# eMWu94/ReMo3D

Hardware: AMD Instinct MI355X
Metric: measurement points/sec (3D benchmark model) (higher is better)
Workload: dtype f64

## Files before the change

include/remo3d_hip_debug.h:

```cpp
#ifndef REMO3D_HIP_DEBUG_H
#define REMO3D_HIP_DEBUG_H

#include "remo3d_hip.h"

#ifdef __cplusplus
extern "C" {
#endif

int remo_debug_stream(remo_ctx_t *ctx, int64_t bytes, double *read_gbs, double *copy_gbs);
int remo_debug_clock(remo_ctx_t *ctx, double *gfma_per_wave);
int remo_debug_cache_gather(remo_ctx_t *ctx, int64_t bytes, double *gbs);
int remo_debug_device(remo_ctx_t *ctx, int64_t *out8);
int remo_debug_xcc(remo_ctx_t *ctx, int32_t *out, int32_t nblocks);


int remo_debug_patch_phases(remo_ctx_t *ctx, remo_batch_t *batch, int32_t fp32 , double *out16);

int remo_debug_patch_phases_p(remo_ctx_t *ctx, remo_batch_t *batch, int32_t fp32, double *out16);

int remo_debug_grid_barrier(remo_ctx_t *ctx, int32_t nblocks, int32_t nbar, double *out3);

int remo_debug_sens_timing(remo_ctx_t *ctx, double *out2);
int remo_debug_sens_group_timing(remo_ctx_t *ctx, double *out4);
int remo_debug_field_timing(remo_ctx_t *ctx, double *out2);
int remo_debug_point_location(remo_ctx_t *ctx);
int remo_debug_direction_bytes(remo_ctx_t *ctx);
int remo_debug_direction_forms(remo_ctx_t *ctx, int64_t n, int64_t nv, int32_t k, int32_t grid, int32_t step, double tol2, const double *r,
                               const float *p, const double *z, const double *dinv, const double *part_even, const double *part_odd,
                               int32_t nb_rz, const double *scal48, float *p_flat, float *p_row, double *scal_flat, double *scal_row);
int remo_debug_vector_heads(remo_ctx_t *ctx, int32_t on, double *out8);
int remo_debug_secondary_timing(remo_ctx_t *ctx, double *ms);
int remo_debug_pairs_timing(remo_ctx_t *ctx, double *out2);
int remo_debug_pair_groups_timing(remo_ctx_t *ctx, double *out4);

int remo_debug_tune(int32_t key, int32_t value);

#ifdef __cplusplus
}
#endif
#endif
```

remo3d_amd/_lib.py:

```python
from __future__ import annotations

import ctypes as C
import os

import numpy as np

_HERE = os.path.dirname(os.path.abspath(__file__))
LIB_PATH = os.environ.get("REMO_LIB") or os.path.join(_HERE, "libremo3d_hip.so")
REMO_MAX_RHS = 8


class RemoMesh(C.Structure):
    _fields_ = [("dim", C.c_int32), ("n_nodes", C.c_int64), ("coords", C.POINTER(C.c_double)),
                ("n_elems", C.c_int64), ("conn", C.POINTER(C.c_int32)), ("mat", C.POINTER(C.c_int32)),
                ("n_bfacets", C.c_int64), ("bconn", C.POINTER(C.c_int32)), ("bdirichlet", C.POINTER(C.c_uint8))]


class RemoOpts(C.Structure):
    _fields_ = [("preconditioner", C.c_int32), ("condense", C.c_int32), ("maxsteps", C.c_int32),
                ("check_every", C.c_int32), ("rtol", C.c_double), ("time_kernels", C.c_int32),
                ("coarse_degree", C.c_int32), ("coarse_ratio", C.c_int32), ("precision", C.c_int32), ("inner_digits", C.c_int32),
                ("serialize_solves", C.c_int32), ("op", C.c_int32), ("coarse", C.c_int32), ("assemble", C.c_int32), ("quadrature", C.c_int32)]


# ... 6 lines not shown
                ("spmv_ms", C.c_double), ("spmv_launches", C.c_int64), ("spmv_bytes", C.c_double),
                ("pcg_steps", C.c_int64), ("spmv_ms_raw", C.c_double), ("event_overhead_ms", C.c_double),
                ("refinement_cycles", C.c_int64), ("op_used", C.c_int32), ("coarse_used", C.c_int32),
                ("assembled", C.c_int32), ("patch_rounds", C.c_int32)]

    def as_dict(self):
        d = {}
        for name, _ in self._fields_:
            v = getattr(self, name)
            d[name] = list(v) if hasattr(v, "__len__") else v
        return d


class RemoJob(C.Structure):
    _dp, _ip = C.POINTER(C.c_double), C.POINTER(C.c_int32)
    _fields_ = [("size", C.c_uint32), ("tensor", C.c_int32), ("n_mat", C.c_int32), ("sigma", _dp),
                ("n_rhs", C.c_int32), ("src_ptr", _ip), ("src_p", _dp), ("src_I", _dp),
                ("eval_ptr", _ip), ("eval_p", _dp), ("u_out", _dp),
                ("n_fun", C.c_int32), ("fun_rhs", _ip), ("fun_ptr", _ip), ("fun_p", _dp), ("fun_w", _dp), ("J_out", _dp), ("dJ_out", _dp),
                ("n_group", C.c_int32), ("group", _ip), ("dJg_out", _dp),
                ("warm", C.c_void_p),
                ("n_pts", C.c_int32), ("pts", _dp), ("n_frhs", C.c_int32), ("field_rhs", _ip), ("u_f", _dp), ("grad_f", _dp), ("J_f", _dp),
                ("elem_f", _ip)]


class RemoJobSecondary(C.Structure):
    _fields_ = RemoJob._fields_ + [("secondary", C.c_int32), ("sec_quad", C.c_int32), ("sec_radius", C.c_double),
                                   ("sec_sigma0", C.POINTER(C.c_double))]


class RemoJobError(C.Structure):
    _fields_ = RemoJobSecondary._fields_ + [("err", C.c_int32), ("err_n_group", C.c_int32), ("err_group", C.POINTER(C.c_int32)),
                                            ("err_out", C.POINTER(C.c_double)), ("errg_out", C.POINTER(C.c_double))]


class RemoJobPairs(C.Structure):
    _fields_ = RemoJobError._fields_ + [("n_pair", C.c_int32), ("pair_reserved", C.c_int32), ("pair_a", C.POINTER(C.c_int32)),
                                        ("pair_b", C.POINTER(C.c_int32)), ("dP_out", C.POINTER(C.c_double))]


class RemoJobPairGroups(C.Structure):
    _fields_ = RemoJobPairs._fields_ + [("pair_n_group", C.c_int32), ("pair_group_reserved", C.c_int32), ("pair_group", C.POINTER(C.c_int32)),
                                        ("dPg_out", C.POINTER(C.c_double))]


EXPORTS = ["remo_abi_version", "remo_opts_default", "remo_ctx_create", "remo_ctx_destroy", "remo_last_error",
           "remo_solve_batch", "remo_solve_batch_tensor", "remo_solve_batch_sens", "remo_solve_batch_sens_tensor", "remo_solve_batch_sens_groups", "remo_solve_batch_sens_groups_tensor",
           "remo_solve_batch_field", "remo_solve_batch_field_tensor", "remo_batch_field", "remo_host_field_element",
           "remo_warm_create", "remo_warm_destroy", "remo_warm_clear", "remo_warm_info", "remo_solve_batch_sens_warm", "remo_solve_batch_sens_warm_tensor", "remo_batch_create", "remo_batch_create_tensor", "remo_batch_run", "remo_batch_fetch", "remo_batch_destroy",
           "remo_batch_eval", "remo_batch_get_system", "remo_batch_get_vectors", "remo_batch_apply_coarse", "remo_batch_spmv",
           "remo_host_element_matrix", "remo_host_element_matrix_tensor", "remo_host_sens_element", "remo_host_factor_error", "remo_host_symbolic",
           "remo_solve_job", "remo_batch_create_job", "remo_host_point_shapes", "remo_host_secondary_element", "remo_host_error_facet", "remo_host_pair_element"]
DEBUG_EXPORTS = ["remo_debug_stream", "remo_debug_clock", "remo_debug_device", "remo_debug_cache_gather", "remo_debug_xcc", "remo_debug_tune", "remo_debug_patch_phases", "remo_debug_patch_phases_p", "remo_debug_grid_barrier", "remo_debug_sens_timing", "remo_debug_sens_group_timing", "remo_debug_field_timing", "remo_debug_point_location", "remo_debug_secondary_timing", "remo_debug_direction_bytes", "remo_debug_pairs_timing", "remo_debug_pair_groups_timing",
                 "remo_debug_direction_forms", "remo_debug_vector_heads"]

JOB_HEAD = ["n_mat", "sigma", "n_rhs", "src_ptr", "src_p", "src_I", "eval_ptr", "eval_p"]
_SENS = ["u_out", "n_fun", "fun_rhs", "fun_ptr", "fun_p", "fun_w"]
LEGACY_MEMBERS = {"": ["u_out"],
                  "_sens": _SENS + ["J_out", "dJ_out"],
                  "_sens_warm": _SENS + ["J_out", "dJ_out", "warm"],
                  "_sens_groups": _SENS + ["n_group", "group", "J_out", "dJ_out", "dJg_out"],
                  "_field": ["u_out", "n_pts", "pts", "n_frhs", "field_rhs", "u_f", "grad_f", "J_f", "elem_f"]}


def legacy_args(job, kind=None):
    return [getattr(job, name) for name in JOB_HEAD + (LEGACY_MEMBERS[kind] if kind is not None else [])]


_lib = None


def load():
    global _lib
    if _lib is not None:
        return _lib
    if not os.path.exists(LIB_PATH):
        raise ImportError(f"{LIB_PATH} is missing: build it with `make -C remo3d_amd/csrc` "
                          "(or __graft_entry__.build()); remo3d_amd has no CPU fallback")
    L = C.CDLL(LIB_PATH)
    dp, ip, i64p, u8p = C.POINTER(C.c_double), C.POINTER(C.c_int32), C.POINTER(C.c_int64), C.POINTER(C.c_uint8)
    vp = C.c_void_p
    L.remo_abi_version.restype = C.c_int
    L.remo_opts_default.argtypes = [C.POINTER(RemoOpts)]
    L.remo_ctx_create.restype = vp
    L.remo_ctx_create.argtypes = [C.c_int]
    L.remo_ctx_destroy.argtypes = [vp]
    L.remo_last_error.restype = C.c_char_p
    L.remo_last_error.argtypes = [vp]
    member = dict(RemoJob._fields_)
    batch_args = [vp, C.POINTER(RemoMesh)] + [member[name] for name in JOB_HEAD]
    for kind, names in LEGACY_MEMBERS.items():
        for entry in (getattr(L, "remo_solve_batch" + kind), getattr(L, "remo_solve_batch" + kind + "_tensor")):
            entry.restype = C.c_int
            entry.argtypes = batch_args + [member[name] for name in names] + [C.POINTER(RemoOpts), C.POINTER(RemoStats)]
    L.remo_warm_create.restype = vp
    L.remo_warm_create.argtypes = [C.c_int]
    L.remo_warm_destroy.restype = None
    L.remo_warm_destroy.argtypes = [vp]
    L.remo_warm_clear.restype = None
    L.remo_warm_clear.argtypes = [vp]
    L.remo_warm_info.restype = C.c_int
    L.remo_warm_info.argtypes = [vp, i64p, ip, i64p, ip]
    L.remo_solve_job.restype = C.c_int
    L.remo_solve_job.argtypes = [vp, C.POINTER(RemoMesh), vp, C.POINTER(RemoOpts), C.POINTER(RemoStats)]
    L.remo_batch_create_job.restype = C.c_int
    L.remo_batch_create_job.argtypes = [vp, C.POINTER(RemoMesh), vp, C.POINTER(vp)]
    L.remo_host_point_shapes.restype = C.c_int
# ... 27 lines not shown
    L.remo_debug_sens_timing.restype = C.c_int
    L.remo_debug_sens_timing.argtypes = [vp, dp]
    L.remo_batch_create.restype = C.c_int
    L.remo_batch_create.argtypes = batch_args + [C.POINTER(vp)]
    L.remo_batch_create_tensor.restype = C.c_int
    L.remo_batch_create_tensor.argtypes = batch_args + [C.POINTER(vp)]
    L.remo_batch_run.restype = C.c_int
    L.remo_batch_run.argtypes = [vp, vp, C.POINTER(RemoOpts), C.POINTER(RemoStats)]
    L.remo_batch_fetch.restype = C.c_int
    L.remo_batch_fetch.argtypes = [vp, vp, dp]
    L.remo_batch_destroy.argtypes = [vp, vp]
    L.remo_batch_eval.restype = C.c_int
    L.remo_batch_eval.argtypes = [vp, vp, C.c_int32, C.c_int32, dp, dp]
    L.remo_batch_get_system.restype = C.c_int
    L.remo_batch_get_system.argtypes = [vp, vp, ip, ip, dp, dp, ip]
    L.remo_batch_get_vectors.restype = C.c_int
    L.remo_batch_get_vectors.argtypes = [vp, vp, dp, dp, ip]
    L.remo_batch_apply_coarse.restype = C.c_int
    L.remo_batch_apply_coarse.argtypes = [vp, vp, C.c_int32, dp, dp, C.c_int32, i64p]
    L.remo_debug_patch_phases.restype = C.c_int
    L.remo_debug_patch_phases.argtypes = [vp, vp, C.c_int32, dp]
    L.remo_debug_patch_phases_p.restype = C.c_int
    L.remo_debug_patch_phases_p.argtypes = [vp, vp, C.c_int32, dp]
    L.remo_debug_grid_barrier.restype = C.c_int
    L.remo_debug_grid_barrier.argtypes = [vp, C.c_int32, C.c_int32, dp]
    L.remo_debug_xcc.restype = C.c_int
    L.remo_debug_xcc.argtypes = [vp, ip, C.c_int32]
    L.remo_debug_cache_gather.restype = C.c_int
    L.remo_debug_cache_gather.argtypes = [vp, C.c_int64, dp]
    L.remo_debug_device.restype = C.c_int
    L.remo_debug_device.argtypes = [vp, i64p]
    L.remo_debug_clock.restype = C.c_int
    L.remo_debug_clock.argtypes = [vp, dp]
    L.remo_debug_stream.restype = C.c_int
    L.remo_debug_stream.argtypes = [vp, C.c_int64, dp, dp]
    L.remo_batch_spmv.restype = C.c_int
    L.remo_batch_spmv.argtypes = [vp, vp, C.c_int32, dp, dp, C.c_int32, dp]
    L.remo_host_element_matrix.restype = C.c_int
    L.remo_host_element_matrix.argtypes = [C.c_int32, dp, C.c_double, dp]
    L.remo_host_element_matrix_tensor.restype = C.c_int
    L.remo_host_element_matrix_tensor.argtypes = [C.c_int32, dp, dp, dp]
    L.remo_host_factor_error.restype = C.c_double
    L.remo_host_symbolic.restype = C.c_int
    L.remo_host_symbolic.argtypes = [C.POINTER(RemoMesh), C.c_int32, i64p, ip, ip, ip]
    L.remo_debug_tune.restype = C.c_int
    L.remo_debug_tune.argtypes = [C.c_int32, C.c_int32]
    fp = C.POINTER(C.c_float)
    if hasattr(L, "remo_debug_direction_forms"):
        L.remo_debug_direction_forms.restype = C.c_int
        L.remo_debug_direction_forms.argtypes = [vp, C.c_int64, C.c_int64, C.c_int32, C.c_int32, C.c_int32, C.c_double, dp, fp, dp, dp, dp, dp,
                                                 C.c_int32, dp, fp, fp, dp, dp]
        L.remo_debug_vector_heads.restype = C.c_int
        L.remo_debug_vector_heads.argtypes = [vp, C.c_int32, dp]
    _lib = L
    return L


def ptr(a, t):
    return a.ctypes.data_as(C.POINTER(t))


def mesh_struct(mesh):
    coords = np.ascontiguousarray(mesh.coords, dtype=np.float64)
    conn = np.ascontiguousarray(mesh.conn, dtype=np.int32)
    mat = np.ascontiguousarray(mesh.mat, dtype=np.int32)
    bconn = np.ascontiguousarray(mesh.bconn, dtype=np.int32).reshape(-1, mesh.dim)
    bdir = np.ascontiguousarray(mesh.bdirichlet, dtype=np.uint8)
    m = RemoMesh(int(mesh.dim), coords.shape[0], ptr(coords, C.c_double), conn.shape[0], ptr(conn, C.c_int32),
                 ptr(mat, C.c_int32), bconn.shape[0], ptr(bconn, C.c_int32), ptr(bdir, C.c_uint8))
    return m, (coords, conn, mat, bconn, bdir)
```

remo3d_amd/csrc/kernels.h:

```cpp
#pragma once
#include <hip/hip_runtime.h>
#include <stdint.h>

#include <type_traits>

#include "elem_access.h"
#include "tune.h"

namespace remo {

constexpr int kMaxPartialBlocks = 1024;
constexpr int kMaxPoints = 256;

template <int V> using int_c = std::integral_constant<int, V>;
template <class F> void for_k(int k, F &&fn) {
    switch (k) {
        case 1: fn(int_c<1>{}); break;
        case 2: fn(int_c<2>{}); break;
        case 3: fn(int_c<3>{}); break;
        case 4: fn(int_c<4>{}); break;
        case 5: fn(int_c<5>{}); break;
        case 6: fn(int_c<6>{}); break;
        case 7: fn(int_c<7>{}); break;
        default: fn(int_c<8>{}); break;
// ... 33 lines not shown
    const float *c32_ell_val = nullptr;
    float *c32_z = nullptr, *c32_res = nullptr, *c32_d[2] = {nullptr, nullptr};
    const AmgT<T> *amg = nullptr;
    const AmgT<float> *amg32 = nullptr;
    bool defer_q = false;
    bool x_in_direction = false;
    bool pq_bins = false;
    const int64_t *x_ev_at = nullptr;
    T *x_ev = nullptr;
    int x_ev_n = 0;
    float *p32 = nullptr;
    PcgProgress *progress;
    int progress_len;
    int nb_spmv, nb_vec;
};
using PcgBuffers = PcgBuffersT<double>;
constexpr int kPqBins = 256;
constexpr int kScalarSlots = 48;
constexpr int kDoneSlot = 4 * 8;

struct PatchTables {
    int64_t nt = 0, n = 0, npatch = 0;
    int E = 0;
    int rows_cap = 0;
    int block = 256;
    int trim = 1;
    int spread = 4;
    const uint16_t *lidx = nullptr;
    const int32_t *pcount = nullptr;
    const int32_t *prow = nullptr;
    const int32_t *pout = nullptr;
    const int32_t *pboff = nullptr;
    int all_slab = 1;
    const int32_t *row4 = nullptr;
    const int32_t *bptr = nullptr;
    const int32_t *bslot = nullptr;
    const double *C = nullptr;
    int64_t nslot_cap = 0;
    int stagger = 0;
    int rounds = 1;
};
template <class T> struct PatchOpT {
    PatchTables t;
    T *Yb = nullptr;
    double *ppart = nullptr;
    int lds_rows = 0;
    bool dot_bins = false;
};
#ifndef REMO_PATCH_PASSES
#define REMO_PATCH_PASSES 12
#endif
constexpr int kPatchPasses = REMO_PATCH_PASSES;
constexpr int kPatchBlock = 256;
inline size_t patch_lds_bytes(int lds_rows, int k) { return size_t(lds_rows + 2) * size_t(k) * 8; }
constexpr size_t kPatchLdsLimit = 63 * 1024;


template <class T> struct CsrViewT {
    int64_t n;
    int64_t nnz;
    const int32_t *rowptr;
    const int32_t *col;
    const T *val;
    int64_t pair_begin = 0, pair_end = 0;
    const PatchOpT<T> *patch = nullptr;
    bool vertex_block_only = false;
};
using CsrView = CsrViewT<double>;

void launch_metric_terms(const ElemMesh &em, int32_t *errflag, hipStream_t s);
void launch_metric_terms_tensor(const ElemMesh &em, int32_t *errflag, hipStream_t s);
void launch_diag_rows(int dim, int64_t row0, int64_t nfree, const int32_t *adjptr, const uint32_t *adj, const double *C, const double *M, double *dinv, hipStream_t s);
void launch_assemble(int dim, bool condense, int64_t nfree, int64_t pair_begin, int64_t pair_end, const int32_t *rowptr, const int32_t *col,
                     const int32_t *adjptr, const uint32_t *adj, const int32_t *eldof, const double *C,
                     const double *M, double *val, double *dinv, hipStream_t s);

int spmv_grid(int64_t n, int lanes_per_row);
int vec_grid(int64_t n);
int choose_lanes_per_row(int64_t n, int64_t nnz);
template <class T> bool patch_applies(const CsrViewT<T> &A, int k);
template <class T> void launch_spmm(const CsrViewT<T> &A, int k, const T *x, T *y, double *part, const double *scal, int nblocks, hipStream_t s, int step = 0, bool defer = false);

template <class T> void launch_patch_spmm(const CsrViewT<T> &A, int k, const T *x, T *y, double *part, const double *scal, int nblocks, hipStream_t s, int step, bool defer);
void launch_patch_spmm_x32(const CsrViewT<double> &A, int k, const float *x, double *part, const double *scal, int nblocks, hipStream_t s, int step);
template <class T> bool pcg_update_folds(const PcgBuffersT<T> &b);

template <class T> void launch_pcg_init(const CsrViewT<T> &A, int k, const T *f, const PcgBuffersT<T> &b, hipStream_t s);
template <class T> void launch_pcg_update(const CsrViewT<T> &A, int k, int step, double tol2, const PcgBuffersT<T> &b, hipStream_t s);
template <class T> void launch_pcg_direction(const CsrViewT<T> &A, int k, int step, double tol2, const PcgBuffersT<T> &b, hipStream_t s, bool add_x = true);
template <class T> void launch_pcg_final(int k, int step, const PcgBuffersT<T> &b, hipStream_t s);
void launch_direction_form(bool flat, int grid, int64_t n, int64_t nv, int k, int step, double tol2, int nb_rz, const double *part_rz_new,
                           double *scal, const double *r, float *p, const double *dinv, double *z, hipStream_t s);
void set_vector_stamps(long long *stamps);
void launch_vblock_bound(int64_t nv, const CsrView &A, const double *dinv, unsigned long long *out_bits, hipStream_t s);
constexpr int kSquareSlots = 512;
void launch_vblock_square(int64_t nv, const CsrView &A, const double *dinv, int32_t *sq_rowptr, int32_t *sq_col, double *sq_a, double *sq_b,
                          int64_t capacity, int32_t *flag, hipStream_t s);
int cheb_grid(int64_t nv);

void launch_barrier_probe(int nblocks, int nbar, unsigned *counter, int *fail, float *buf, int *mismatch, hipStream_t s);
constexpr int kEllWidth = 24;
void launch_vblock_ell(int64_t nv, const int32_t *rowptr, const int32_t *col, const double *val, int32_t *ecol, int32_t *tail, double *eval64,
                       float *eval32, hipStream_t s);


void launch_to_float(int64_t n, const double *src, float *dst, hipStream_t s);
void launch_vblock_compact(int64_t nv, const CsrView &A, int32_t *vb_rowptr, int32_t *vb_col, double *vb_val, int64_t capacity, int32_t *flag,
// ... 21 lines not shown
```

remo3d_amd/csrc/patch.h:

```cpp
#pragma once
#include "kernels.h"
#include "symbolic_gpu.h"

namespace remo {

size_t patch_arena_bytes(int64_t nt, int64_t n_max, int kmax);
void build_patch_tables(Arena &ar, hipStream_t s, const DeviceSymbolic &sy, const double *C, int kmax, int rounds, PatchTables &out, int32_t *flag_and_max);
int patch_rounds(int kmax, int wanted);
int patch_elements_per_group(int kmax, int rounds);
void set_patch_stamps(long long *device_buffer);

}
```

remo3d_amd/csrc/patch.hip:

```cpp
#include <hip/hip_runtime.h>
#include <limits.h>

#include <rocprim/device/device_scan.hpp>

#include "kernels.h"
#include "kutil.h"
#include "patch.h"
#include <stdexcept>
#include <type_traits>
#include "symbolic_gpu.h"
#include "wave_util.h"

#define REMO_ELEM_NS elem_tables_patch
#include "build/elem_apply.inc"

namespace remo {

namespace {

constexpr int kPatchDotBlocks = 32;
constexpr uint32_t kSlotBits = 13;
constexpr uint64_t kNoRow = uint64_t(0x7FFFFFFF);

__global__ void __launch_bounds__(256) k_patch_row_slots(int64_t n, int E, const int32_t *__restrict__ adjptr, const uint32_t *__restrict__ adj,
// ... 74 lines not shown
        if (lidx[j] == 0xFFFF) lidx[j] = z;
}

__global__ void __launch_bounds__(256) k_patch_slots(int E, int rows_cap, const int32_t *__restrict__ pcount, const int32_t *__restrict__ pboff,
                                                     const int32_t *__restrict__ prow, int32_t *__restrict__ pout, const int32_t *__restrict__ adjptr,
                                                     const uint32_t *__restrict__ adj, const int32_t *__restrict__ bptr, int32_t *__restrict__ bslot,
                                                     int32_t *__restrict__ row4) {
    const int64_t p = blockIdx.x;
    const int mp = pcount[p] < rows_cap ? pcount[p] : rows_cap;
    for (int m = threadIdx.x; m < mp; m += 256) {
        const int32_t row = prow[p * rows_cap + m], slot = pboff[p] + m;
        int32_t last = -1, rank = 0;
        for (int32_t a = adjptr[row]; a < adjptr[row + 1]; ++a) {
            const int32_t q = int32_t((adj[a] >> 5) / uint32_t(E));
            if (q >= p) break;
            rank += q != last;
            last = q;
        }
        pout[p * rows_cap + m] = slot;
        bslot[bptr[row] + rank] = slot;
        const int32_t cnt = bptr[row + 1] - bptr[row];
        if (rank < 3 || (rank == 3 && cnt <= 4)) row4[int64_t(row) * 4 + rank] = slot;
        else if (rank == 3) row4[int64_t(row) * 4 + 3] = -2;
    }
}

template <class T> __device__ __forceinline__ void lds_add(T *p, T v) {
    (void)__hip_atomic_fetch_add(p, v, __ATOMIC_RELAXED, __HIP_MEMORY_SCOPE_WORKGROUP);
}

#ifndef REMO_LEAN_WAVES
#define REMO_LEAN_WAVES 5
#endif
constexpr int kPatchPasses2 = 20;
template <class T, int K, int MODE = 0, bool LEAN = false, int ROUNDS = 1, class TX = T>
__global__ void __launch_bounds__(kPatchBlock, (LEAN ? REMO_LEAN_WAVES : 1)) k_patch_apply(PatchTables tb, int rows, const TX *__restrict__ x, T *__restrict__ y, T *__restrict__ Yb,
                                                     double *__restrict__ ppart, const double *__restrict__ scal, int step, long long *__restrict__ stamps,
                                                     double *__restrict__ pbins) {
    static_assert(std::is_same<TX, T>::value || (std::is_same<TX, float>::value && std::is_same<T, double>::value && MODE == 0 && !LEAN),
                  "an x narrower than the rest: fp32 into the fp64 product, plain order");
    (void)y;
    int done_word = 0;
    if (scal) done_word = load_as_vector(reinterpret_cast<const int *>(scal + kDoneSlot));
#define REMO_STAMP(k) if constexpr (MODE == 4) { if (threadIdx.x == 0) stamps[(int64_t(blockIdx.x) << 3) + (k)] = __builtin_readcyclecounter(); }
    REMO_STAMP(0)
    constexpr int NL = K;
    static_assert(ROUNDS == 1 || (ROUNDS == 2 && MODE == 0 && !LEAN), "two rounds: the plain order of the product only");
    constexpr int U = ROUNDS == 2 ? kPatchPasses2 : kPatchPasses;
    constexpr int BLK = kPatchBlock;
    constexpr int EK = BLK / K;
    constexpr uint32_t S = sizeof(T), SX = sizeof(TX);
    extern __shared__ double lds_raw[];
    TX *xs = reinterpret_cast<TX *>(lds_raw);
    __shared__ double smem[16 * K];
    const int tid = threadIdx.x;
    const int64_t per = (tb.npatch + 7) >> 3;
    const int64_t p = int64_t(blockIdx.x & 7) * per + int64_t(blockIdx.x >> 3);
    if (p >= tb.npatch) return;
    const int32_t *prow = tb.prow + p * tb.rows_cap;
    const int el = tid / NL, c0 = tid - el * NL;
    const int32_t off_mask = tid < EK * K ? 0 : int32_t(0x80000000);
    const rsrc_t rpr = make_rsrc(prow, uint64_t(tb.rows_cap) * 4);
    int32_t r0[U];
    const int rows_own_v = load_as_vector(tb.pcount + p);
    const int slab0_v = load_as_vector(tb.pboff + p);
#pragma unroll
    for (int u = 0; u < U; ++u) {
        int32_t t[1];
        buf_load<int32_t, 1>(rpr, off_mask == 0 ? uint32_t(el + EK * u) * 4u : kOutOfRange, t);
        r0[u] = t[0];
    }
    const int R = tb.spread > 1 ? tb.spread : 1;
    const int EL = ROUNDS == 2 ? (tb.E >> 1) : tb.E;
    const int run = el % R, base = EL / R, extra = EL % R;
    const int elp = R > 1 ? (run * base + (run < extra ? run : extra) + el / R) : el;
    const int64_t e = p * tb.E + elp;
    const bool active = el < EL && e < tb.nt;
    const int64_t eB = e + EL;
    const bool activeB = ROUNDS == 2 && el < EL && eB < tb.nt;
    uint32_t li[10];
    double cm[6];
#pragma unroll
    for (int q = 0; q < 10; ++q) li[q] = 0u;
#pragma unroll
    for (int q = 0; q < 6; ++q) cm[q] = 0.0;
    const rsrc_t rli = make_rsrc(tb.lidx, uint64_t(tb.nt) * 40), rcm = make_rsrc(tb.C, uint64_t(tb.nt) * 48);
    buf_load<uint32_t, 10>(rli, active ? uint32_t(e) * 40u : kOutOfRange, li);
    if constexpr (!(LEAN && MODE != 2)) buf_load<double, 6>(rcm, active ? uint32_t(e) * 48u : kOutOfRange, cm);
    uint32_t liB[ROUNDS == 2 ? 10 : 1];
    double cmB[ROUNDS == 2 ? 6 : 1];
    if constexpr (ROUNDS == 2) {
#pragma unroll
        for (int q = 0; q < 10; ++q) liB[q] = 0u;
#pragma unroll
        for (int q = 0; q < 6; ++q) cmB[q] = 0.0;
        buf_load<uint32_t, 10>(rli, activeB ? uint32_t(eB) * 40u : kOutOfRange, liB);
        buf_load<double, 6>(rcm, activeB ? uint32_t(eB) * 48u : kOutOfRange, cmB);
    }
    const int rows_own = __builtin_amdgcn_readfirstlane(rows_own_v);
    if (__builtin_amdgcn_readfirstlane(done_word) != 0 && __builtin_amdgcn_readfirstlane(done_word) <= step) return;
    const int rows_p = (tb.trim && rows_own < rows) ? rows_own : rows;
    const int npass = (rows_p + EK - 1) / EK;
    REMO_STAMP(1)
    const rsrc_t rx = make_rsrc(x, uint64_t(tb.n) * K * SX);
    const uint32_t slack = uint32_t((rows + 1) * K + c0);
#define REMO_PASSES_UP_TO_12(fn)                                                                                          \
        case 1: fn(std::integral_constant<int, 1>{}, 0); break;   case 2: fn(std::integral_constant<int, 2>{}, 0); break;   \
        case 3: fn(std::integral_constant<int, 3>{}, 0); break;   case 4: fn(std::integral_constant<int, 4>{}, 0); break;   \
        case 5: fn(std::integral_constant<int, 5>{}, 0); break;   case 6: fn(std::integral_constant<int, 6>{}, 0); break;   \
        case 7: fn(std::integral_constant<int, 7>{}, 0); break;   case 8: fn(std::integral_constant<int, 8>{}, 0); break;   \
        case 9: fn(std::integral_constant<int, 9>{}, 0); break;   case 10: fn(std::integral_constant<int, 10>{}, 0); break; \
        case 11: fn(std::integral_constant<int, 11>{}, 0); break; case 12: fn(std::integral_constant<int, 12>{}, 0); break;
#define REMO_PASSES(fn)                                                                                                   \
    if constexpr (ROUNDS == 2) {                                                                                          \
        switch (npass) {                                                                                                  \
            REMO_PASSES_UP_TO_12(fn)                                                                                      \
            case 13: fn(std::integral_constant<int, 13>{}, 0); break; case 14: fn(std::integral_constant<int, 14>{}, 0); break; \
            case 15: fn(std::integral_constant<int, 15>{}, 0); break; case 16: fn(std::integral_constant<int, 16>{}, 0); break; \
            case 17: fn(std::integral_constant<int, 17>{}, 0); break; case 18: fn(std::integral_constant<int, 18>{}, 0); break; \
            case 19: fn(std::integral_constant<int, 19>{}, 0); break; case 20: fn(std::integral_constant<int, 20>{}, 0); break; \
            default:                                                                                                      \
                for (int m0 = 0; m0 < rows_p; m0 += U * EK) fn(std::integral_constant<int, U>{}, m0);                     \
        }                                                                                                                 \
    } else {                                                                                                              \
        switch (npass) {                                                                                                  \
            REMO_PASSES_UP_TO_12(fn)                                                                                      \
            default:                                                                                                      \
                for (int m0 = 0; m0 < rows_p; m0 += U * EK) fn(std::integral_constant<int, U>{}, m0);                     \
        }                                                                                                                 \
    }
    static_assert(kPatchPasses == 12 && kPatchPasses2 == 20, "REMO_PASSES lists the cases 1 .. U");
    auto stage = [&](auto np_c, int m0) {
        constexpr int NP = decltype(np_c)::value;
        int32_t r[NP];
        TX v[NP][1];
        if (m0 == 0) {
#pragma unroll
            for (int u = 0; u < NP; ++u) r[u] = r0[u];
        } else {
#pragma unroll
            for (int u = 0; u < NP; ++u) {
                int32_t t[1];
                buf_load<int32_t, 1>(rpr, off_mask == 0 ? uint32_t(m0 + el + EK * u) * 4u : kOutOfRange, t);
                r[u] = t[0];
            }
        }
#pragma unroll
        for (int u = 0; u < NP; ++u) r[u] = (off_mask == 0 && m0 + el + EK * u < rows_own) ? r[u] : -1;
#pragma unroll
        for (int u = 0; u < NP; ++u)
            buf_load<TX, 1>(rx, r[u] >= 0 ? __umul24(uint32_t(r[u]), K * SX) + uint32_t(c0) * SX : kOutOfRange, v[u]);
#pragma unroll
        for (int u = 0; u < NP; ++u) xs[r[u] >= 0 ? uint32_t((m0 + el + EK * u) * K + c0) : slack] = v[u][0];
    };
    REMO_PASSES(stage)
    if (tid < 2 * K) xs[rows * K + tid] = TX(0);
    __syncthreads();
    REMO_STAMP(2)
    double d0 = 0.0;
    double *ya = lds_raw;
#define REMO_PATCH_L(i) ((li[(i) >> 1] >> (16 * ((i) & 1))) & 0xFFFFu)
    if constexpr (LEAN && MODE != 2) {
        typedef const T __attribute__((address_space(4))) *ctab_t;
        ctab_t tgi = (ctab_t)ElemTables2<T>::grad_in(), tdo = (ctab_t)ElemTables2<T>::div_out();
        if constexpr (sizeof(T) == 8) { asm volatile("" : "+s"(tgi)); asm volatile("" : "+s"(tdo)); }
        T g[30];
#define REMO_PATCH_XL(i) xs[REMO_PATCH_L(i) * K + c0]
#define REMO_BAR_ON __builtin_amdgcn_sched_barrier(0);
#define REMO_BAR_OFF
        if constexpr (sizeof(T) == 4) { REMO_ELEM_GRAD_IN(T, REMO_PATCH_XL, g, tgi, REMO_BAR_ON) }
        else { REMO_ELEM_GRAD_IN(T, REMO_PATCH_XL, g, tgi, REMO_BAR_OFF) }
#undef REMO_PATCH_XL
#pragma unroll
        for (int j = 0; j < 30; ++j) asm volatile("" : "+v"(g[j]));
        __builtin_amdgcn_sched_barrier(0);
        if (active) {
            const double *ce = tb.C + e * 6;
#pragma unroll
            for (int q = 0; q < 6; ++q) cm[q] = ce[q];
        }
        __syncthreads();
        REMO_STAMP(3)
        for (int j = 2 * tid; j < rows_p * K; j += 2 * BLK) { ya[j] = 0.0; ya[j + 1] = 0.0; }
        if (tid < K) ya[rows * K + tid] = 0.0;
        __syncthreads();
        REMO_STAMP(4)
        if (active) {
            const T c11 = T(cm[0]), c12 = T(cm[1]), c13 = T(cm[2]), c22 = T(cm[3]), c23 = T(cm[4]), c33 = T(cm[5]);
            T dd = T(0);
#pragma unroll
            for (int m = 0; m < 10; ++m) {
                const T g1 = g[m], g2 = g[10 + m], g3 = g[20 + m];
                const T h1 = c11 * g1 + c12 * g2 + c13 * g3, h2 = c12 * g1 + c22 * g2 + c23 * g3, h3 = c13 * g1 + c23 * g2 + c33 * g3;
                dd += g1 * h1 + g2 * h2 + g3 * h3;
                g[m] = h1; g[10 + m] = h2; g[20 + m] = h3;
            }
            d0 = double(dd);
            if constexpr (sizeof(T) == 8) {
                const uint32_t *pl2 = reinterpret_cast<const uint32_t *>(tb.lidx + e * 20);
#pragma unroll
                for (int q = 0; q < 10; ++q) li[q] = __builtin_nontemporal_load(pl2 + q);
            }
#define REMO_PATCH_EMIT(i, v) { if constexpr (MODE == 1) ya[REMO_PATCH_L(i) * K + c0] = double(v); else lds_add(ya + REMO_PATCH_L(i) * K + c0, double(v)); }
            if constexpr (sizeof(T) == 4) { REMO_ELEM_DIV_OUT(T, g, tdo, REMO_PATCH_EMIT, REMO_BAR_ON) }
            else { REMO_ELEM_DIV_OUT(T, g, tdo, REMO_PATCH_EMIT, REMO_BAR_OFF) }
#undef REMO_PATCH_EMIT
#undef REMO_BAR_ON
#undef REMO_BAR_OFF
        }
    } else if constexpr (ROUNDS == 2) {
        typedef const T __attribute__((address_space(4))) *ctab_t;
        ctab_t tgrad = (ctab_t)ElemTables<T>::grad(), tdiv = (ctab_t)ElemTables<T>::div();
        if constexpr (sizeof(T) == 8) { asm volatile("" : "+s"(tgrad)); asm volatile("" : "+s"(tdiv)); }
        auto element = [&](const T (&xe)[20], const double (&ce)[6], T (&ye)[20]) -> double {
            const T c11 = T(ce[0]), c12 = T(ce[1]), c13 = T(ce[2]), c22 = T(ce[3]), c23 = T(ce[4]), c33 = T(ce[5]);
            T g[30];
            REMO_ELEM_GRAD(T, xe, g, tgrad)
            T dd = T(0);
#pragma unroll
            for (int m = 0; m < 10; ++m) {
                const T g1 = g[m], g2 = g[10 + m], g3 = g[20 + m];
                const T h1 = c11 * g1 + c12 * g2 + c13 * g3, h2 = c12 * g1 + c22 * g2 + c23 * g3, h3 = c13 * g1 + c23 * g2 + c33 * g3;
                dd += g1 * h1 + g2 * h2 + g3 * h3;
                g[m] = h1; g[10 + m] = h2; g[20 + m] = h3;
            }
            REMO_ELEM_DIV(T, g, ye, tdiv)
            return double(dd);
        };
        auto emit = [&](int64_t ee, const T (&ye)[20]) {
            uint32_t lq[10];
            const uint32_t *pl2 = reinterpret_cast<const uint32_t *>(tb.lidx + ee * 20);
#pragma unroll
            for (int q = 0; q < 10; ++q) lq[q] = __builtin_nontemporal_load(pl2 + q);
#pragma unroll
            for (int i = 0; i < 20; ++i) lds_add(ya + ((lq[i >> 1] >> (16 * (i & 1))) & 0xFFFFu) * K + c0, double(ye[i]));
        };
        T yA[20], xB[20];
        double dA = 0.0;
        if (active) {
            T xA[20];
#pragma unroll
            for (int i = 0; i < 20; ++i) xA[i] = T(xs[REMO_PATCH_L(i) * K + c0]);
            dA = element(xA, cm, yA);
#pragma unroll
            for (int i = 0; i < 20; ++i) asm volatile("" : "+v"(yA[i]));
        }
        if (activeB) {
#pragma unroll
            for (int i = 0; i < 20; ++i) xB[i] = T(xs[((liB[i >> 1] >> (16 * (i & 1))) & 0xFFFFu) * K + c0]);
        }
        __syncthreads();
        REMO_STAMP(3)
        for (int j = 2 * tid; j < rows_p * K; j += 2 * BLK) { ya[j] = 0.0; ya[j + 1] = 0.0; }
        if (tid < K) ya[rows * K + tid] = 0.0;
        __syncthreads();
        REMO_STAMP(4)
        if (active) emit(e, yA);
        d0 = dA;
        if (activeB) {
            T yB[20];
            d0 += element(xB, cmB, yB);
            emit(eB, yB);
        }
    } else {
    T xv[20];
    if (active) {
#pragma unroll
        for (int i = 0; i < 20; ++i) xv[i] = T(xs[REMO_PATCH_L(i) * K + c0]);
    }
    __syncthreads();
    REMO_STAMP(3)
    for (int j = 2 * tid; j < rows_p * K; j += 2 * BLK) { ya[j] = 0.0; ya[j + 1] = 0.0; }
    if (tid < K) ya[rows * K + tid] = 0.0;
    __syncthreads();
    REMO_STAMP(4)
    if (active) {
        const T c11 = T(cm[0]), c12 = T(cm[1]), c13 = T(cm[2]), c22 = T(cm[3]), c23 = T(cm[4]), c33 = T(cm[5]);
        T g[30], yv[20];
        if constexpr (MODE == 2) {
#pragma unroll
            for (int i = 0; i < 20; ++i) yv[i] = xv[i] * c11;
        } else {
            typedef const T __attribute__((address_space(4))) *ctab_t;
            ctab_t tgrad = (ctab_t)ElemTables<T>::grad(), tdiv = (ctab_t)ElemTables<T>::div();
            if constexpr (sizeof(T) == 8) { asm volatile("" : "+s"(tgrad)); asm volatile("" : "+s"(tdiv)); }
            REMO_ELEM_GRAD(T, xv, g, tgrad)
            T dd = T(0);
#pragma unroll
            for (int m = 0; m < 10; ++m) {
                const T g1 = g[m], g2 = g[10 + m], g3 = g[20 + m];
                const T h1 = c11 * g1 + c12 * g2 + c13 * g3, h2 = c12 * g1 + c22 * g2 + c23 * g3, h3 = c13 * g1 + c23 * g2 + c33 * g3;
                dd += g1 * h1 + g2 * h2 + g3 * h3;
                g[m] = h1; g[10 + m] = h2; g[20 + m] = h3;
            }
            d0 = double(dd);
            REMO_ELEM_DIV(T, g, yv, tdiv)
        }
        {
            const uint32_t *pl2 = reinterpret_cast<const uint32_t *>(tb.lidx + e * 20);
// ... 194 lines not shown
    if constexpr (K == 5) {
        if (!launched && tb.rounds == 1 && mode >= 1 && mode <= 3 + (g_patch_stamps ? 1 : 0)) {
            launched = true;
            if (mode == 1) launch(k_patch_apply<T, 5, 1>);
            else if (mode == 2) launch(k_patch_apply<T, 5, 2>);
            else if (mode == 3) launch(k_patch_apply<T, 5, 3>);
            else launch(k_patch_apply<T, 5, 4>);
        }
    }
    if (!launched && tb.rounds == 1 && ((lean == 1) != (sizeof(T) == 4)) && lean >= 0) {
        if (sizeof(T) == 4) launch(k_patch_apply<T, K, 0>); else launch(k_patch_apply<T, K, 0, true>);
        launched = true;
    }
#endif
    if (!launched) {
        if constexpr (sizeof(T) == 4) {
            if (tb.rounds != 1) throw std::logic_error("patch operator: tables of two rounds in fp32 storage (they are built for fp64 solves only)");
            launch(k_patch_apply<T, K, 0, true>);
        } else {
            if (tb.rounds == 2) launch(k_patch_apply<T, K, 0, false, 2>);
            else launch(k_patch_apply<T, K, 0>);
        }
    }
    if (bins) return;
    if (part && defer) {
        hipLaunchKernelGGL(k_patch_dot<K>, dim3(nb < kPatchDotBlocks ? nb : kPatchDotBlocks), dim3(256), 0, s, tb.npatch, (const double *)P.ppart, part, scal, step);
        return;
    }
    if (part) hipLaunchKernelGGL((k_patch_reduce<T, K, true>), dim3(nb), dim3(256), 0, s, A.n, tb.npatch, tb.bptr, tb.bslot, (const T *)P.Yb, y, (const double *)P.ppart, part, scal, step);
    else hipLaunchKernelGGL((k_patch_reduce<T, K, false>), dim3(nb), dim3(256), 0, s, A.n, tb.npatch, tb.bptr, tb.bslot, (const T *)P.Yb, y, (const double *)nullptr, part, scal, step);
}

template <class T> void launch_patch_spmm(const CsrViewT<T> &A, int k, const T *x, T *y, double *part, const double *scal, int nb, hipStream_t s, int step, bool defer) {
    for_k(k, [&](auto kc) { constexpr int K = decltype(kc)::value; patch_dispatch<T, K>(A, x, y, part, scal, step, nb, s, defer); });
}
template <int K> static void patch_dispatch_x32(const CsrViewT<double> &A, const float *x, double *part, const double *scal, int step, int nb, hipStream_t s) {
    const PatchOpT<double> &P = *A.patch;
    const PatchTables &tb = P.t;
    const int64_t per = (tb.npatch + 7) / 8;
    double *bins = P.dot_bins ? part + (step & 1) * (kPqBins * 8) : nullptr;
    const size_t bytes = patch_lds_bytes(P.lds_rows, K);
    if (tb.rounds == 2)
        hipLaunchKernelGGL((k_patch_apply<double, K, 0, false, 2, float>), dim3(int(per * 8)), dim3(kPatchBlock), bytes, s, tb, P.lds_rows, x, (double *)nullptr, P.Yb, P.ppart, scal, step, (long long *)nullptr, bins);
    else
        hipLaunchKernelGGL((k_patch_apply<double, K, 0, false, 1, float>), dim3(int(per * 8)), dim3(kPatchBlock), bytes, s, tb, P.lds_rows, x, (double *)nullptr, P.Yb, P.ppart, scal, step, (long long *)nullptr, bins);
    if (!bins) hipLaunchKernelGGL(k_patch_dot<K>, dim3(nb < kPatchDotBlocks ? nb : kPatchDotBlocks), dim3(256), 0, s, tb.npatch, (const double *)P.ppart, part, scal, step);
}

void launch_patch_spmm_x32(const CsrViewT<double> &A, int k, const float *x, double *part, const double *scal, int nb, hipStream_t s, int step) {
    if (!patch_applies(A, k) || !part) throw std::logic_error("patch operator on an fp32 direction: no patch tables for this batch");
    for_k(k, [&](auto kc) { constexpr int K = decltype(kc)::value; patch_dispatch_x32<K>(A, x, part, scal, step, nb, s); });
}

template void launch_patch_spmm<double>(const CsrViewT<double> &, int, const double *, double *, double *, const double *, int, hipStream_t, int, bool);
template void launch_patch_spmm<float>(const CsrViewT<float> &, int, const float *, float *, double *, const double *, int, hipStream_t, int, bool);

}
```

remo3d_amd/csrc/remo_debug.hip:

```cpp
#include <limits.h>

#include <algorithm>
#include <vector>

#include "../../include/remo3d_hip_debug.h"
#include "remo_internal.h"
#include "patch.h"

using namespace remo;

namespace remo {
Tune g_tune;
}

extern "C" {

namespace {
__global__ void __launch_bounds__(256) k_stream_read(const double2 *__restrict__ x, int64_t n2, double *__restrict__ out) {
    double a = 0.0, b = 0.0;
    for (int64_t i = int64_t(blockIdx.x) * blockDim.x + threadIdx.x; i < n2; i += int64_t(gridDim.x) * blockDim.x) {
        const double2 v = x[i];
        a += v.x; b += v.y;
    }
    a += b;
// ... 240 lines not shown
};

int patch_probe_check(remo_ctx *ctx, remo_batch *b) {
    if (!b->has_system || b->run_id != ctx->run_id || !b->A.patch) return fail(ctx, REMO_ERR_ARG, "the last run on this batch did not use the patch operator");
    if (b->patch64.t.rounds != 1) return fail(ctx, REMO_ERR_ARG, "the batch's patch tables hold two elements per lane: set remo_debug_tune key 40 to 1 and run the batch again");
    if (PatchProbe::k * b->patch64.t.E > kPatchBlock) return fail(ctx, REMO_ERR_ARG, "the batch's patch tables are laid out for fewer than 5 columns");
    return REMO_OK;
}
}
#endif

int remo_debug_patch_phases(remo_ctx_t *ctx, remo_batch_t *b, int32_t fp32, double *out16) {
    if (!ctx || !b || !out16) return REMO_ERR_ARG;
#ifndef REMO_PROBES
    (void)fp32;
    return fail(ctx, REMO_ERR_ARG, "remo_debug_patch_phases: the library was built without -DREMO_PROBES (make -C remo3d_amd/csrc probes)");
#else
    if (int rc = patch_probe_check(ctx, b)) return rc;
    struct PersistOff { int was = g_tune.patch_persist; PersistOff() { g_tune.patch_persist = 0; } ~PersistOff() { g_tune.patch_persist = was; } } persist_off;
    try {
        HIP_TRY(hipSetDevice(ctx->device));
        const int64_t grid = (b->patch64.t.npatch + 7) / 8 * 8;
        std::vector<long long> h;
        {
            PatchProbe pr(ctx, b, fp32 != 0, size_t(grid) * 8);
            pr.stamped_runs();
            for (int mode = 0; mode <= 3; ++mode) {
                g_tune.patch_mode = mode;
                out16[10 + mode] = pr.timed_us();
            }
            g_tune.patch_mode = 0;
            h = pr.stamps();
        }
        for (int i = 0; i < 10; ++i) out16[i] = 0.0;
        long long lo = LLONG_MAX, hi = 0;
        int64_t cnt = 0;
        for (int64_t w = 0; w < grid; ++w) {
            const long long *s8 = h.data() + w * 8;
            if (s8[0] == 0 || s8[7] == 0) continue;
            for (int q = 0; q < 7; ++q) out16[q] += double(s8[q + 1] - s8[q]);
            out16[7] += double(s8[7] - s8[0]);
            lo = std::min(lo, s8[0]); hi = std::max(hi, s8[7]);
            ++cnt;
        }
        for (int q = 0; q < 8; ++q) out16[q] /= double(cnt > 0 ? cnt : 1);
        out16[8] = double(hi - lo);
        out16[9] = double(cnt);
        return REMO_OK;
    } catch (const std::exception &ex) {
        g_tune.patch_mode = 0; set_patch_stamps(nullptr);
        return fail(ctx, REMO_ERR_DEVICE, ex.what());
    }
#endif
}

int remo_debug_patch_phases_p(remo_ctx_t *ctx, remo_batch_t *b, int32_t fp32, double *out16) {
    if (!ctx || !b || !out16) return REMO_ERR_ARG;
#ifndef REMO_PROBES
    (void)fp32;
    return fail(ctx, REMO_ERR_ARG, "remo_debug_patch_phases_p: the library was built without -DREMO_PROBES (make -C remo3d_amd/csrc probes)");
#else
    if (int rc = patch_probe_check(ctx, b)) return rc;
    const int64_t slots = 8192;
    try {
        HIP_TRY(hipSetDevice(ctx->device));
        std::vector<long long> h;
        double us = 0.0;
        {
            PatchProbe pr(ctx, b, fp32 != 0, size_t(slots) * 12);
            pr.stamped_runs();
            us = pr.timed_us();
            h = pr.stamps();
        }
        for (int i = 0; i < 16; ++i) out16[i] = 0.0;
        double patches = 0, wgs = 0, longest = 0;
        for (int64_t w = 0; w < slots; ++w) {
            const long long *s12 = h.data() + w * 12;
            if (s12[10] <= 0) continue;
            double tot = 0;
            for (int q = 0; q < 10; ++q) { out16[q] += double(s12[q]); tot += double(s12[q]); }
            patches += double(s12[10]); wgs += 1; longest = std::max(longest, tot);
        }
        for (int q = 0; q < 10; ++q) out16[q] /= (patches > 0 ? patches : 1);
        out16[10] = patches; out16[11] = wgs; out16[12] = longest; out16[13] = us;
        return REMO_OK;
    } catch (const std::exception &ex) {
        g_tune.patch_mode = 0; set_patch_stamps(nullptr);
        return fail(ctx, REMO_ERR_DEVICE, ex.what());
    }
#endif
}

int remo_debug_direction_forms(remo_ctx_t *ctx, int64_t n, int64_t nv, int32_t k, int32_t grid, int32_t step, double tol2, const double *r,
                               const float *p, const double *z, const double *dinv, const double *part_even, const double *part_odd,
                               int32_t nb_rz, const double *scal48, float *p_flat, float *p_row, double *scal_flat, double *scal_row) {
    if (!ctx || n < 1 || nv < 0 || nv > n || k < 1 || k > 8 || grid < 1 || grid > kMaxPartialBlocks || step < 0 || nb_rz < 0 || nb_rz > kMaxPartialBlocks ||
        !r || !p || !dinv || (nv > 0 && !z) || !part_even || !part_odd || !scal48 || !p_flat || !p_row || !scal_flat || !scal_row)
        return REMO_ERR_ARG;
    if (uint64_t(n) * uint64_t(k) * 8 >= 0xFFFFF000ull) return fail(ctx, REMO_ERR_ARG, "remo_debug_direction_forms: n k sizeof(double) must stay below 4 GB (the flat form's range)");
    try {
        HIP_TRY(hipSetDevice(ctx->device));
        const size_t N = size_t(n) * k, NV = size_t(nv) * k, NP = size_t(nb_rz > 0 ? nb_rz : 1) * k;
        DeviceTemp tmp;
        double *dr = tmp.alloc<double>(N), *dz = tmp.alloc<double>(NV + 2), *dd = tmp.alloc<double>(n), *dpart = tmp.alloc<double>(2 * NP),
               *dscal = tmp.alloc<double>(48);
        float *dp = tmp.alloc<float>(N);
// ... 168 lines not shown
```

remo3d_amd/solver.py:

```python
from __future__ import annotations

import ctypes as C
from typing import Optional

import numpy as np

from . import _lib
from ._lib import RemoOpts, RemoStats, ptr

REMO_OK = 0
REMO_NOT_CONVERGED = 1
REMO_ERR_ARG = -1


class RemoError(RuntimeError):
    def __init__(self, code, msg):
        super().__init__(f"libremo3d_hip error {code}: {msg}")
        self.code = code


def make_opts(preconditioner="multigrid", condense=True, maxsteps=1000, rtol=1e-8, check_every=5,
              time_kernels=False, coarse_degree=0, coarse_ratio=0, precision="fp64", inner_digits=0,
              serialize_solves=False, op="auto", coarse="auto", quadrature="exact", assemble="auto") -> RemoOpts:
    L = _lib.load()
# ... 387 lines not shown
            n_group = int(groups.max(initial=-1)) + 1 if n_group is None else int(n_group)
            pg = (groups, n_group)
        out = self._one_shot("_sens", mesh, sigma, sources, evals, opts, raise_on_error, list(functionals) if functionals else [], pairs=pairs,
                             pair_groups=pg)
        if functionals:
            return out
        potentials, dP, st, rc = out[0], out[3], out[-2], out[-1]
        dPg = out[4] if pg is not None else None
        if far_field is not None and rc >= 0:
            ref = far_field_reference(mesh, sigma, float(far_field), *(pg or ()))
            c, dc = ref[0], ref[1]
            k = 2.0 if int(mesh.dim) == 3 else 1.0
            total = [float(np.sum(I)) for (_, I) in sources]
            potentials = [u + k * total[r] * c for r, u in enumerate(potentials)]
            if len(dP):
                pa, pb = _pair_arrays(pairs)
                kII = (k * np.array(total)[pa] * np.array(total)[pb]).reshape((-1,) + (1,) * dc.ndim)
                dP = dP + kII * dc[None]
                if pg is not None:
                    dPg = dPg + kII * ref[2][None]
        if pg is not None:
            return potentials, dP, dPg, st, rc
        return potentials, dP, st, rc

    def pairs_timing(self):
        out = np.zeros(2)
        self._L.remo_debug_pairs_timing(self._h, ptr(out, C.c_double))
        return float(out[0]), int(out[1])

    def pair_groups_timing(self):
        out = np.zeros(4)
        self._L.remo_debug_pair_groups_timing(self._h, ptr(out, C.c_double))
        return float(out[0]), float(out[1]), float(out[2]), int(out[3])

    def solve_batch_field(self, mesh, sigma, sources, evals, points, field_rhs=None, opts: Optional[RemoOpts] = None, raise_on_error=True):
        return self._one_shot("_field", mesh, sigma, sources, evals, opts, raise_on_error, points=points, field_rhs=field_rhs)

    def field_timing(self):
        out = np.zeros(2)
        self._L.remo_debug_field_timing(self._h, ptr(out, C.c_double))
        return float(out[0]), float(out[1])

    def secondary_timing(self) -> float:
        ms = C.c_double(0.0)
        self._L.remo_debug_secondary_timing(self._h, C.byref(ms))
        return float(ms.value)

    def point_location(self) -> int:
        return int(self._L.remo_debug_point_location(self._h))

    def direction_bytes(self) -> int:
        return int(self._L.remo_debug_direction_bytes(self._h))

    def sens_group_timing(self):
        out = np.zeros(4)
        self._L.remo_debug_sens_group_timing(self._h, ptr(out, C.c_double))
        return tuple(float(v) for v in out)

    def sens_timing(self):
        out = np.zeros(2)
        self._L.remo_debug_sens_timing(self._h, ptr(out, C.c_double))
        return float(out[0]), float(out[1])

    def batch(self, mesh, sigma, sources, evals, secondary=None) -> "Batch":
        return Batch(self, mesh, sigma, sources, evals, secondary)


class Batch:

    def __init__(self, ctx: Context, mesh, sigma, sources, evals, secondary=None):
        self.ctx = ctx
        self._L = ctx._L
        job = secondary is not None or _off_axis([z for (z, _) in sources], evals)
        if secondary is not None and not _secondary_members(secondary, len(sources))[3]:
            raise RemoError(REMO_ERR_ARG, "secondary: sigma0 must be positive and finite (None: the conductivity at the source)")
        (handle, ms, j), _, tensor, self._eval_ptr, keep = _batch_args(ctx._h, mesh, sigma, sources, evals, job, secondary)
        h = C.c_void_p()
        if job:
            rc = self._L.remo_batch_create_job(handle, ms, C.byref(j), C.byref(h))
        else:
            rc = (self._L.remo_batch_create_tensor if tensor else self._L.remo_batch_create)(handle, ms, *_lib.legacy_args(j), C.byref(h))
        if rc != 0:
            raise RemoError(rc, ctx.last_error())
        self._h = h
        self.dim = int(mesh.dim)
        self.n_rhs = len(sources)
        self.stats = None

    def run(self, opts: Optional[RemoOpts] = None, raise_on_error=True, ctx: Optional["Context"] = None):
        st = RemoStats()
        o = opts if opts is not None else make_opts()
        if ctx is not None:
            self.ctx = ctx
        rc = self._L.remo_batch_run(self.ctx._h, self._h, C.byref(o), C.byref(st))
        self.stats = st.as_dict()
        if rc < 0 and raise_on_error:
            raise RemoError(rc, self.ctx.last_error())
        return rc

    def fetch(self):
        eval_ptr = self._eval_ptr
        out = np.full(int(eval_ptr[-1]), np.nan)
        rc = self._L.remo_batch_fetch(self.ctx._h, self._h, ptr(out, C.c_double))
        if rc != 0:
            raise RemoError(rc, self.ctx.last_error())
        return [out[eval_ptr[k]:eval_ptr[k + 1]] for k in range(self.n_rhs)]
# ... 163 lines not shown
```

Measured before the change: 193.4.

## Alias patch smem into dynamic LDS and defer second-round loads to cut pressure

In the two-round patch apply kernel, the static 16*K shared scratch is dropped and aliased onto the dynamic LDS buffer, whose minimum size is raised to four rows so it can hold the scratch. The second-round index and coefficient loads are moved from the prologue to just before their use, with only a one-word cache warm-up issued early. Both changes aim to lower LDS and register footprint so more workgroups fit per CU, at the cost of exposing some load latency later in the kernel. A debug occupancy query export is also added.

```diff
diff --git a/include/remo3d_hip_debug.h b/include/remo3d_hip_debug.h
--- a/include/remo3d_hip_debug.h
+++ b/include/remo3d_hip_debug.h
@@ -15,6 +15,8 @@
 
 
 int remo_debug_patch_phases(remo_ctx_t *ctx, remo_batch_t *batch, int32_t fp32 , double *out16);
+
+int remo_debug_patch_occupancy(remo_ctx_t *ctx, int32_t lds_rows, int32_t k, int32_t rounds, int32_t x32, int32_t *out);
 
 int remo_debug_patch_phases_p(remo_ctx_t *ctx, remo_batch_t *batch, int32_t fp32, double *out16);
 
diff --git a/remo3d_amd/_lib.py b/remo3d_amd/_lib.py
--- a/remo3d_amd/_lib.py
+++ b/remo3d_amd/_lib.py
@@ -82,7 +82,7 @@
            "remo_host_element_matrix", "remo_host_element_matrix_tensor", "remo_host_sens_element", "remo_host_factor_error", "remo_host_symbolic",
            "remo_solve_job", "remo_batch_create_job", "remo_host_point_shapes", "remo_host_secondary_element", "remo_host_error_facet", "remo_host_pair_element"]
 DEBUG_EXPORTS = ["remo_debug_stream", "remo_debug_clock", "remo_debug_device", "remo_debug_cache_gather", "remo_debug_xcc", "remo_debug_tune", "remo_debug_patch_phases", "remo_debug_patch_phases_p", "remo_debug_grid_barrier", "remo_debug_sens_timing", "remo_debug_sens_group_timing", "remo_debug_field_timing", "remo_debug_point_location", "remo_debug_secondary_timing", "remo_debug_direction_bytes", "remo_debug_pairs_timing", "remo_debug_pair_groups_timing",
-                 "remo_debug_direction_forms", "remo_debug_vector_heads"]
+                 "remo_debug_direction_forms", "remo_debug_vector_heads", "remo_debug_patch_occupancy"]
 
 JOB_HEAD = ["n_mat", "sigma", "n_rhs", "src_ptr", "src_p", "src_I", "eval_ptr", "eval_p"]
 _SENS = ["u_out", "n_fun", "fun_rhs", "fun_ptr", "fun_p", "fun_w"]
@@ -216,6 +216,9 @@
                                                  C.c_int32, dp, fp, fp, dp, dp]
         L.remo_debug_vector_heads.restype = C.c_int
         L.remo_debug_vector_heads.argtypes = [vp, C.c_int32, dp]
+    if hasattr(L, "remo_debug_patch_occupancy"):
+        L.remo_debug_patch_occupancy.restype = C.c_int
+        L.remo_debug_patch_occupancy.argtypes = [vp, C.c_int32, C.c_int32, C.c_int32, C.c_int32, ip]
     _lib = L
     return L
 
diff --git a/remo3d_amd/csrc/kernels.h b/remo3d_amd/csrc/kernels.h
--- a/remo3d_amd/csrc/kernels.h
+++ b/remo3d_amd/csrc/kernels.h
@@ -109,7 +109,7 @@
 #endif
 constexpr int kPatchPasses = REMO_PATCH_PASSES;
 constexpr int kPatchBlock = 256;
-inline size_t patch_lds_bytes(int lds_rows, int k) { return size_t(lds_rows + 2) * size_t(k) * 8; }
+inline size_t patch_lds_bytes(int lds_rows, int k) { return size_t(lds_rows + 2 > 4 ? lds_rows + 2 : 4) * size_t(k) * 8; }
 constexpr size_t kPatchLdsLimit = 63 * 1024;
 
 
diff --git a/remo3d_amd/csrc/patch.h b/remo3d_amd/csrc/patch.h
--- a/remo3d_amd/csrc/patch.h
+++ b/remo3d_amd/csrc/patch.h
@@ -8,6 +8,7 @@
 void build_patch_tables(Arena &ar, hipStream_t s, const DeviceSymbolic &sy, const double *C, int kmax, int rounds, PatchTables &out, int32_t *flag_and_max);
 int patch_rounds(int kmax, int wanted);
 int patch_elements_per_group(int kmax, int rounds);
+int patch_apply_occupancy(int k, int rounds, bool x32, int lds_rows);
 void set_patch_stamps(long long *device_buffer);
 
 }
diff --git a/remo3d_amd/csrc/patch.hip b/remo3d_amd/csrc/patch.hip
--- a/remo3d_amd/csrc/patch.hip
+++ b/remo3d_amd/csrc/patch.hip
@@ -150,7 +150,12 @@
     constexpr uint32_t S = sizeof(T), SX = sizeof(TX);
     extern __shared__ double lds_raw[];
     TX *xs = reinterpret_cast<TX *>(lds_raw);
-    __shared__ double smem[16 * K];
+    double *smem;
+    if constexpr (ROUNDS == 2) smem = lds_raw;
+    else {
+        __shared__ double smem_static[16 * K];
+        smem = smem_static;
+    }
     const int tid = threadIdx.x;
     const int64_t per = (tb.npatch + 7) >> 3;
     const int64_t p = int64_t(blockIdx.x & 7) * per + int64_t(blockIdx.x >> 3);
@@ -185,15 +190,14 @@
     const rsrc_t rli = make_rsrc(tb.lidx, uint64_t(tb.nt) * 40), rcm = make_rsrc(tb.C, uint64_t(tb.nt) * 48);
     buf_load<uint32_t, 10>(rli, active ? uint32_t(e) * 40u : kOutOfRange, li);
     if constexpr (!(LEAN && MODE != 2)) buf_load<double, 6>(rcm, active ? uint32_t(e) * 48u : kOutOfRange, cm);
-    uint32_t liB[ROUNDS == 2 ? 10 : 1];
-    double cmB[ROUNDS == 2 ? 6 : 1];
+    uint32_t warmB[2] = {0u, 0u};
     if constexpr (ROUNDS == 2) {
-#pragma unroll
-        for (int q = 0; q < 10; ++q) liB[q] = 0u;
-#pragma unroll
-        for (int q = 0; q < 6; ++q) cmB[q] = 0.0;
-        buf_load<uint32_t, 10>(rli, activeB ? uint32_t(eB) * 40u : kOutOfRange, liB);
-        buf_load<double, 6>(rcm, activeB ? uint32_t(eB) * 48u : kOutOfRange, cmB);
+        uint32_t t[1];
+        const uint32_t eB0 = uint32_t(p * tb.E + EL), at = uint32_t(tid) * 16u;
+        buf_load<uint32_t, 1>(rli, at < uint32_t(EL) * 40u ? eB0 * 40u + at : kOutOfRange, t);
+        warmB[0] = t[0];
+        buf_load<uint32_t, 1>(rcm, at < uint32_t(EL) * 48u ? eB0 * 48u + at : kOutOfRange, t);
+        warmB[1] = t[0];
     }
     const int rows_own = __builtin_amdgcn_readfirstlane(rows_own_v);
     if (__builtin_amdgcn_readfirstlane(done_word) != 0 && __builtin_amdgcn_readfirstlane(done_word) <= step) return;
@@ -252,6 +256,7 @@
         for (int u = 0; u < NP; ++u) xs[r[u] >= 0 ? uint32_t((m0 + el + EK * u) * K + c0) : slack] = v[u][0];
     };
     REMO_PASSES(stage)
+    if constexpr (ROUNDS == 2) asm volatile("" : : "v"(warmB[0]), "v"(warmB[1]));
     if (tid < 2 * K) xs[rows * K + tid] = TX(0);
     __syncthreads();
     REMO_STAMP(2)
@@ -343,6 +348,15 @@
 #pragma unroll
             for (int i = 0; i < 20; ++i) asm volatile("" : "+v"(yA[i]));
         }
+        __builtin_amdgcn_sched_barrier(0);
+        uint32_t liB[10];
+        double cmB[6];
+#pragma unroll
+        for (int q = 0; q < 10; ++q) liB[q] = 0u;
+#pragma unroll
+        for (int q = 0; q < 6; ++q) cmB[q] = 0.0;
+        buf_load<uint32_t, 10>(rli, activeB ? uint32_t(eB) * 40u : kOutOfRange, liB);
+        buf_load<double, 6>(rcm, activeB ? uint32_t(eB) * 48u : kOutOfRange, cmB);
         if (activeB) {
 #pragma unroll
             for (int i = 0; i < 20; ++i) xB[i] = T(xs[((liB[i >> 1] >> (16 * (i & 1))) & 0xFFFFu) * K + c0]);
@@ -643,6 +657,24 @@
     for_k(k, [&](auto kc) { constexpr int K = decltype(kc)::value; patch_dispatch_x32<K>(A, x, part, scal, step, nb, s); });
 }
 
+int patch_apply_occupancy(int k, int rounds, bool x32, int lds_rows) {
+    int n = -1;
+    for_k(k, [&](auto kc) {
+        constexpr int K = decltype(kc)::value;
+        const size_t bytes = patch_lds_bytes(lds_rows, K);
+        hipError_t rc;
+        if (rounds == 2) {
+            if (x32) rc = hipOccupancyMaxActiveBlocksPerMultiprocessor(&n, k_patch_apply<double, K, 0, false, 2, float>, kPatchBlock, bytes);
+            else rc = hipOccupancyMaxActiveBlocksPerMultiprocessor(&n, k_patch_apply<double, K, 0, false, 2>, kPatchBlock, bytes);
+        } else {
+            if (x32) rc = hipOccupancyMaxActiveBlocksPerMultiprocessor(&n, k_patch_apply<double, K, 0, false, 1, float>, kPatchBlock, bytes);
+            else rc = hipOccupancyMaxActiveBlocksPerMultiprocessor(&n, k_patch_apply<double, K, 0>, kPatchBlock, bytes);
+        }
+        if (rc != hipSuccess) n = -1;
+    });
+    return n;
+}
+
 template void launch_patch_spmm<double>(const CsrViewT<double> &, int, const double *, double *, double *, const double *, int, hipStream_t, int, bool);
 template void launch_patch_spmm<float>(const CsrViewT<float> &, int, const float *, float *, double *, const double *, int, hipStream_t, int, bool);
 
diff --git a/remo3d_amd/csrc/remo_debug.hip b/remo3d_amd/csrc/remo_debug.hip
--- a/remo3d_amd/csrc/remo_debug.hip
+++ b/remo3d_amd/csrc/remo_debug.hip
@@ -316,6 +316,20 @@
         return fail(ctx, REMO_ERR_DEVICE, ex.what());
     }
 #endif
+}
+
+int remo_debug_patch_occupancy(remo_ctx_t *ctx, int32_t lds_rows, int32_t k, int32_t rounds, int32_t x32, int32_t *out) {
+    if (!ctx || !out || k < 1 || k > 8 || (rounds != 1 && rounds != 2) || lds_rows < 0) return REMO_ERR_ARG;
+    if (patch_lds_bytes(lds_rows, k) > kPatchLdsLimit) return fail(ctx, REMO_ERR_ARG, "remo_debug_patch_occupancy: more rows than a workgroup's LDS holds");
+    try {
+        HIP_TRY(hipSetDevice(ctx->device));
+        const int n = patch_apply_occupancy(k, rounds, x32 != 0, lds_rows);
+        if (n < 0) return fail(ctx, REMO_ERR_DEVICE, "hipOccupancyMaxActiveBlocksPerMultiprocessor failed");
+        *out = n;
+        return REMO_OK;
+    } catch (const std::exception &ex) {
+        return fail(ctx, REMO_ERR_DEVICE, ex.what());
+    }
 }
 
 int remo_debug_patch_phases_p(remo_ctx_t *ctx, remo_batch_t *b, int32_t fp32, double *out16) {
diff --git a/remo3d_amd/solver.py b/remo3d_amd/solver.py
--- a/remo3d_amd/solver.py
+++ b/remo3d_amd/solver.py
@@ -463,6 +463,13 @@
     def direction_bytes(self) -> int:
         return int(self._L.remo_debug_direction_bytes(self._h))
 
+    def patch_occupancy(self, lds_rows: int, k: int, rounds: int = 2, x32: bool = True) -> int:
+        out = C.c_int32(-1)
+        rc = self._L.remo_debug_patch_occupancy(self._h, int(lds_rows), int(k), int(rounds), 1 if x32 else 0, C.byref(out))
+        if rc != 0:
+            raise RemoError(rc, self.last_error())
+        return int(out.value)
+
     def sens_group_timing(self):
         out = np.zeros(4)
         self._L.remo_debug_sens_group_timing(self._h, ptr(out, C.c_double))
```

After: 195.7, median of 6. +1.2%, better.
